# Caxson/mere-fusion

Hardware: AMD Instinct MI355X
Metric: lip-sync frames/sec @256x256 (higher is better)
Workload: dtype bf16x3+f16q; 1 GPU; MuseTalk step 256x256: pe(audio) + UNet(t=0) + VAE decode to uint8 frames, batch=8 latents + Whisper chunks per GPU, inputs resident in HBM (BASELINE.json configs[2]); assumed MuseTalk-v1 / sd-vae-ft-mse architecture, seeded random-init weights; batch_per_gpu=8, parallelism=1 independent replicas, sessions sharded by GPU, no collective

## Files before the change

### mere-fusion_amd/csrc/mf_conv.h

```cpp
#pragma once
#include "mf_common.h"
#include <map>
#include <vector>
#include <utility>

struct ActBuf {
    int C = 0, H = 0, W = 0, halo = 0;
    bf16_t* hi = nullptr;
    bf16_t* lo = nullptr;
    int Hp() const { return H + 2 * halo; }
    int Wp() const { return W + 2 * halo; }
    int64_t per_batch() const { return (int64_t)Hp() * Wp() * C; }
};

struct ActView {
    const ActBuf* buf = nullptr;
    int coff = 0;
    int C = 0;
};

#define MF_MAX_PHASE 9

struct ConvPhase {
    int goff_begin;
// ... 4 lines not shown
    int64_t ws_off;
};

struct ConvArgs {
    const bf16_t* x_hi; const bf16_t* x_lo;
    const bf16_t* w_hi; const bf16_t* w_lo;
    const float* bias;
    const bf16_t* r_hi; const bf16_t* r_lo;
    bf16_t* y_hi; bf16_t* y_lo;
    const int* goff;
    int M, N, Npad;
    int HqWq, Wq;
    uint32_t dv_hw_mul, dv_hw_shr, dv_w_mul, dv_w_shr;
    uint32_t dv_t_mul, dv_t_shr, dv_s_mul, dv_s_shr;
    int64_t xb; int xi, xj;
    int64_t yb; int yi, yj;
    int64_t rb; int ri, rj;
    int act;
    int res_after_act;
    int tiles_m, tiles_n;
    unsigned long long* dbg;
    int m_fastest;
    int ld;
    int wide_store;
    int goff_total;
    int zgroups, zheads;
    int64_t zx_b, zx_h, zw, zy_b, zy_h;
    float* ws;
    int64_t ws_split, wsb; int wsi, wsj;
    double* gn_out; int gn_out_cpg, gn_out_groups;
    double* ln_out; const double* ln_in; const float* ln_cs; float ln_inv_c, ln_eps;
    ConvPhase ph[MF_MAX_PHASE];
};

struct HaloArgs {
    const bf16_t* x_hi; const bf16_t* x_lo;
    const bf16_t* w_hi; const bf16_t* w_lo;
    const float* bias;
    const bf16_t* r_hi; const bf16_t* r_lo;
    bf16_t* y_hi; bf16_t* y_lo;
    int batch, H, W, N, Npad, n_slices;
    int in_halo, in_hp, in_wp, x_ld;
    int64_t xb;
    int64_t yb; int yi, yj;
    int64_t rb; int ri, rj;
    int act;
    int res_from_halo;
    int patches_x, patches_per_img, n_patches, tiles_n;
    float* ws; int64_t ws_split; int nsplit;
    unsigned long long* dbg;
    int q;
    double* gn_out; int gn_out_cpg, gn_out_groups;
    int wide_store;
};
struct HaloTile { int ph, bn, wgm, wgn; };

struct ThinArgs {
    const bf16_t* x_hi; const bf16_t* x_lo;
    const bf16_t* w;
    const float* bias;
    bf16_t* y_hi; bf16_t* y_lo;
    int batch, H, W, N;
    int pad, in_halo, in_hp, in_wp, x_ld;
    int64_t xb, yb; int yi, yj;
    int act;
};
bool mf_thin_supported(int k, int stride, int cin, int cout);
int mf_thin_nks(int k, int cin);
void mf_thin_pack(const float* w, const float* scale, int cout, int cin, int k, bool x3, std::vector<bf16_t>& dst);
int mf_thin_launch(const ThinArgs& a, int k, int stride, int cin, int cout, bool x3, hipStream_t s);
HaloTile mf_halo_pick_tile(int H, int W, int N, int batch, int cin = 0);
int mf_halo_launch(const HaloArgs& a, const HaloTile& t, bool x3, hipStream_t s);
HaloTile mf_halo_w_pick_tile(int H, int W, int N, int batch, int cin = 0);
int mf_halo_w_launch(const HaloArgs& a, const HaloTile& t, bool x3, hipStream_t s, int phase = -1);
struct ConvTile { int bm, bn, wgm, wgn, nsplit; };
struct ConvTuned { ConvTile tile; int ld; };

struct ConvPlan {
    mf_conv2d_desc d{};
    int precision = 0;
    int cin_pad = 0;
    int out_h = 0, out_w = 0;
    int Hq = 0, Wq = 0;
    int nphase = 1;
    int Npad = 0;
    int BK = 64;
    bf16_t* w_hi = nullptr;
    bf16_t* w_lo = nullptr;
    float* bias = nullptr;
    int* goff = nullptr;
    double* out_stats = nullptr; int out_stats_groups = 0;
    const float* ln_gamma = nullptr; const float* ln_beta = nullptr;
    float* ln_cs = nullptr; const double* ln_in = nullptr; float ln_eps = 1e-5f;
    double* ln_out = nullptr;
    bool q_small_maps = false;
    bool q = false;
    bool halo = false;
    bool thin = false;
    bf16_t* up_hi = nullptr;
    bf16_t* up_lo = nullptr;
    ConvPlan* alt = nullptr;
    int n_slices = 0;
    int groups_cap = 1;
    hipEvent_t prof_mid = nullptr;
    float* ws = nullptr;
    int64_t ws_cap = 0;
    std::vector<void*> retired;
    struct Tap {
        int dy, dx;
        std::vector<std::pair<int, int>> src;
    };
    std::vector<std::vector<Tap>> phase_taps;
    std::vector<int> phase_oy, phase_ox;
    int out_step = 1;
    int in_step_h = 1, in_step_w = 1;
    int in_halo_need = 0;
    ConvPhase ph[MF_MAX_PHASE]{};
    int goff_total = 0;
    int bound_in_ld = -1, bound_in_wp = -1;
    std::map<int, ConvTuned> tuned;
};

int mf_conv_plan_create(ConvPlan* p, const mf_conv2d_desc& d, const float* weight, const float* bias,
                        const float* bn_gamma, const float* bn_beta, const float* bn_mean,
                        const float* bn_var, int precision);
void mf_conv_plan_destroy(ConvPlan* p);

int mf_conv_bind(ConvPlan* p, const ActBuf& in);

struct ConvLaunchCfg { int family; ConvTile tile; int ld, bk, nphase, stats; bool pinned; };
int mf_conv_resolve(const ConvPlan* p, int batch, int tokens, int stats_groups, ConvLaunchCfg* c);
bool mf_conv_tuned_valid(const ConvTuned& c, int precision, int act);
int mf_conv_pin(ConvPlan* p, int batch, const ConvTuned& c);
void mf_conv_kernel_name(const ConvPlan* p, int batch, char* buf, int cap);
ConvTile mf_conv_pick_tile(const ConvPlan* p, int batch);
int mf_conv_tune(ConvPlan* p, const ActView& in, const ActView& out, const ActView& res, int batch, hipStream_t stream);
int mf_conv_tune_lookup(ConvPlan* p, const ActView& in, int batch);
bool mf_autotune_enabled();
double mf_conv_flops(const ConvPlan* p, int batch);

struct GroupedGemm {
    const bf16_t* x_hi; const bf16_t* x_lo; int64_t zx_b, zx_h; int x_row;
    bf16_t* y_hi; bf16_t* y_lo; int64_t zy_b, zy_h; int y_row;
    int M, groups, heads;
};
int mf_gemm_grouped_launch(ConvPlan* p, const GroupedGemm& g, hipStream_t stream);

int mf_q_split_count(const ConvPlan* p, int batch);
// ... 6 lines not shown
```

### mere-fusion_amd/csrc/mf_conv.hip

```cpp
#include "mf_conv.h"
#include <dlfcn.h>
#include <cmath>
#include <cstdlib>
#include <cstring>
#include <algorithm>
#include <map>
#include <set>
#include <string>
#include <type_traits>

typedef __attribute__((ext_vector_type(8))) __bf16 bf16x8;
typedef __attribute__((ext_vector_type(4))) float f32x4;
typedef __attribute__((ext_vector_type(4))) unsigned int u32x4;
typedef __attribute__((ext_vector_type(8))) _Float16 f16x8;
typedef __attribute__((ext_vector_type(8))) int i32x8;
typedef __attribute__((ext_vector_type(4))) int i32x4;

template <int BK>
__device__ __forceinline__ int swz(int row) {
    return BK == 32 ? (((row >> 2) & 1) << 1) : (((row >> 1) & 3) << 1);
}
template <int BK>
__device__ __forceinline__ int tile_off(int row, int kg) {
    return row * (BK * 2) + ((kg ^ swz<BK>(row)) << 4);
// ... 1747 lines not shown
        ha.x_hi = ib.hi + in.coff; ha.x_lo = x3 ? ib.lo + in.coff : nullptr;
        ha.w_hi = p->w_hi; ha.w_lo = p->w_lo; ha.bias = p->bias;
        ha.batch = batch; ha.H = p->out_h; ha.W = p->out_w; ha.N = p->d.cout; ha.Npad = p->Npad; ha.n_slices = p->n_slices;
        ha.in_halo = ib.halo; ha.in_hp = ib.Hp(); ha.in_wp = ib.Wp(); ha.x_ld = ib.C; ha.xb = ib.per_batch();
        const int64_t yb0 = ((int64_t)ob.halo * ob.Wp() + ob.halo) * ob.C + out.coff;
        ha.y_hi = ob.hi + yb0; ha.y_lo = x3 ? ob.lo + yb0 : nullptr;
        ha.yb = ob.per_batch(); ha.yi = ob.Wp() * ob.C; ha.yj = ob.C;
        if (res.buf) {
            const ActBuf& rb = *res.buf;
            MF_REQUIRE(rb.H == p->out_h && rb.W == p->out_w && res.C == p->d.cout, "conv: residual view does not match the output");
            if (res.buf == in.buf && res.coff == in.coff && p->d.cin == p->d.cout) {
                ha.res_from_halo = 1;
            } else {
                const int64_t rb0 = ((int64_t)rb.halo * rb.Wp() + rb.halo) * rb.C + res.coff;
                ha.r_hi = rb.hi + rb0; ha.r_lo = x3 ? rb.lo + rb0 : nullptr;
                ha.rb = rb.per_batch(); ha.ri = rb.Wp() * rb.C; ha.rj = rb.C;
            }
        }
        ha.act = p->d.act;
        if (cfg.family == MF_CONV_FAMILY_F16Q) {
            MF_REQUIRE(!ha.res_from_halo, "conv (f16q): residual-from-input is not built for this format");
            if (cfg.stats == MF_CONV_STATS_EPILOGUE) {
                ha.gn_out = p->out_stats; ha.gn_out_cpg = p->d.cout / p->out_stats_groups; ha.gn_out_groups = p->out_stats_groups;
                *stats_done = true;
            }
            ha.wide_store = out.coff % 8 == 0 && ob.C % 8 == 0 && p->d.cout % 32 == 0;
            const HaloTile qtile{16, 128, 4, 2};
            const int ns = cfg.tile.nsplit;
            if (ns > 1) {
                const int64_t per_split = (int64_t)batch * p->out_h * p->out_w * p->d.cout;
                const int64_t need = per_split * ns;
                if (need > p->ws_cap) {
                    if (p->ws) { p->retired.push_back(p->ws); p->ws = nullptr; p->ws_cap = 0; }
                    MF_HIP(hipMalloc(&p->ws, need * sizeof(float)));
                    p->ws_cap = need;
                }
                HaloArgs hs = ha;
                hs.ws = p->ws; hs.ws_split = per_split; hs.nsplit = ns;
                hs.gn_out = nullptr;
                *stats_done = false;
                int rc = mf_halo_w_launch(hs, qtile, true, stream);
                if (rc) return rc;
                ConvArgs e{};
                e.ws = p->ws; e.ws_split = per_split; e.bias = p->bias; e.N = p->d.cout; e.act = p->d.act;
                e.y_hi = ha.y_hi; e.y_lo = ha.y_lo; e.yb = ha.yb; e.yi = ha.yi; e.yj = ha.yj;
                e.r_hi = ha.r_hi; e.r_lo = ha.r_lo; e.rb = ha.rb; e.ri = ha.ri; e.rj = ha.rj;
                const int64_t total = (int64_t)batch * p->out_h * p->out_w * (p->d.cout / 4);
                MF_REQUIRE(total < 0x7fffffffll, "conv: split-K combine over %lld channel quads (32-bit thread index)", (long long)total);
                if (launch_combine_stats(p, e, ns, p->out_h, p->out_w, batch, stream)) *stats_done = true;
                else hipLaunchKernelGGL(k_splitk_epilogue, dim3((unsigned)((total + 255) / 256)), dim3(256), 0, stream, e, ns, p->out_h, p->out_w, (int)total, epi_div(e, p->out_h, p->out_w));
                MF_HIP(hipGetLastError());
                return MF_OK;
            }
            return mf_halo_w_launch(ha, qtile, true, stream);
        }
        if (cfg.family == MF_CONV_FAMILY_HALO_W) return mf_halo_w_launch(ha, HaloTile{cfg.tile.bm, cfg.tile.bn, cfg.tile.wgm, cfg.tile.wgn}, x3, stream);
        {
            const int ns = cfg.tile.nsplit;
            if (cfg.family == MF_CONV_FAMILY_HALO_W_SPLIT) {
                const int64_t per_split = (int64_t)batch * p->out_h * p->out_w * p->d.cout;
                const int64_t need = per_split * ns;
                if (need > p->ws_cap) {
                    if (p->ws) { p->retired.push_back(p->ws); p->ws = nullptr; p->ws_cap = 0; }
                    MF_HIP(hipMalloc(&p->ws, need * sizeof(float)));
                    p->ws_cap = need;
                }
                HaloArgs hs = ha;
                hs.ws = p->ws; hs.ws_split = per_split; hs.nsplit = ns;
                hs.res_from_halo = 0;
                int rc = mf_halo_w_launch(hs, HaloTile{16, 256, 2, 4}, x3, stream);
                if (rc) return rc;
                ConvArgs e{};
                e.ws = p->ws; e.ws_split = per_split; e.bias = p->bias; e.N = p->d.cout; e.act = p->d.act;
                e.y_hi = ha.y_hi; e.y_lo = ha.y_lo; e.yb = ha.yb; e.yi = ha.yi; e.yj = ha.yj;
                if (res.buf) {
                    const ActBuf& rb = *res.buf;
                    const int64_t rb0 = ((int64_t)rb.halo * rb.Wp() + rb.halo) * rb.C + res.coff;
                    e.r_hi = rb.hi + rb0; e.r_lo = x3 ? rb.lo + rb0 : nullptr;
                    e.rb = rb.per_batch(); e.ri = rb.Wp() * rb.C; e.rj = rb.C;
                }
                const int64_t total = (int64_t)batch * p->out_h * p->out_w * (p->d.cout / 4);
                MF_REQUIRE(total < 0x7fffffffll, "conv: split-K combine over %lld channel quads (32-bit thread index)", (long long)total);
                if (launch_combine_stats(p, e, ns, p->out_h, p->out_w, batch, stream)) *stats_done = true;
                else hipLaunchKernelGGL(k_splitk_epilogue, dim3((unsigned)((total + 255) / 256)), dim3(256), 0, stream, e, ns, p->out_h, p->out_w, (int)total, epi_div(e, p->out_h, p->out_w));
                MF_HIP(hipGetLastError());
                return MF_OK;
            }
        }
        if (cfg.family == MF_CONV_FAMILY_TWIN) {
            p->alt->prof_mid = p->prof_mid;
            p->alt->out_stats = p->out_stats; p->alt->out_stats_groups = p->out_stats_groups;
            const int rc = conv_launch_impl(p->alt, in, out, res, batch, stream, 0, stats_done);
            p->alt->prof_mid = nullptr;
            return rc;
        }
        return mf_halo_launch(ha, HaloTile{cfg.tile.bm, cfg.tile.bn, cfg.tile.wgm, cfg.tile.wgn}, x3, stream);
    }

    if (cfg.family == MF_CONV_FAMILY_F16Q) {
        MF_REQUIRE(ib.halo >= 1 && !res.buf, "conv (f16q): upsample path needs an input halo and no residual");
        HaloArgs ha{};
        ha.q = 1;
        ha.x_hi = ib.hi + in.coff; ha.x_lo = ib.lo + in.coff;
        ha.bias = p->bias;
        ha.batch = batch; ha.H = p->d.in_h; ha.W = p->d.in_w; ha.N = p->d.cout; ha.Npad = p->Npad; ha.n_slices = p->n_slices;
        ha.in_halo = ib.halo; ha.in_hp = ib.Hp(); ha.in_wp = ib.Wp(); ha.x_ld = ib.C; ha.xb = ib.per_batch();
// ... 471 lines not shown
```

### mere-fusion_amd/csrc/mf_conv_halo2.hip

```cpp
#include "mf_conv.h"
#include <cstdlib>
#include <cstdio>
#include <vector>
#include <algorithm>
#include <type_traits>

typedef __attribute__((ext_vector_type(8))) __bf16 bf16x8;
typedef __attribute__((ext_vector_type(4))) float f32x4;
typedef __attribute__((ext_vector_type(8))) _Float16 f16x8;
typedef __attribute__((ext_vector_type(8))) int i32x8;
typedef __attribute__((ext_vector_type(4))) int i32x4;

namespace {

constexpr int PW = 16;

template <int CK>
__device__ __forceinline__ int hswz(int hx) {
    return CK == 32 ? (((hx >> 2) & 1) << 1) : (((hx >> 1) & 3) << 1);
}

__device__ __forceinline__ int qswz(int r) { return ((r >> 2) & 1) * 3; }

__device__ __forceinline__ float hbf2f(uint32_t h16) { return __uint_as_float(h16 << 16); }
// ... 499 lines not shown
                __syncthreads();
            }
            wbuf ^= 1;
        }
    }

    if (dbg && threadIdx.x == 0) dbg[2] = __builtin_amdgcn_s_memtime();
    float gs[Q ? FN : 1], gq[Q ? FN : 1];
#pragma unroll
    for (int i = 0; i < (Q ? FN : 1); ++i) { gs[i] = 0.f; gq[i] = 0.f; }
    constexpr int FME = SP ? FM / 2 : FM;
    const int erow0 = row0 + (SP && !cons ? FM / 2 : 0);
    if constexpr (SP) {
        f32x4* xch = reinterpret_cast<f32x4*>(smem);
        __syncthreads();
        if (cons) {
#pragma unroll
            for (int i = 0; i < FN; ++i)
#pragma unroll
                for (int jj = 0; jj < FME; ++jj) xch[((wave * FN + i) * FME + jj) * 64 + lane] = acc[i][FME + jj];
        }
        __syncthreads();
        if (!cons) {
#pragma unroll
            for (int i = 0; i < FN; ++i)
#pragma unroll
                for (int jj = 0; jj < FME; ++jj) acc[i][jj] = xch[(((wave - NW) * FN + i) * FME + jj) * 64 + lane];
        }
    }
    if (a.ws) {
#pragma unroll
        for (int j = 0; j < FME; ++j) {
            const int oy = y0 + erow0 + j, ox = x0 + fr;
            if (oy >= a.H || ox >= a.W) continue;
            float* wo = a.ws + (int64_t)blockIdx.y * a.ws_split + (((int64_t)b * a.H + oy) * a.W + ox) * a.N;
#pragma unroll
            for (int i = 0; i < FN; ++i) {
                const int c = n0 + cn0 + i * 16 + fk * 4;
                if (c >= a.N) continue;
                *reinterpret_cast<float4*>(wo + c) = make_float4(acc[i][j][0], acc[i][j][1], acc[i][j][2], acc[i][j][3]);
            }
        }
        return;
    }
    float4 bq[FN];
#pragma unroll
    for (int i = 0; i < FN; ++i) {
        int c = n0 + cn0 + i * 16 + fk * 4;
        c = c < a.Npad - 3 ? c : a.Npad - 4;
        bq[i] = *reinterpret_cast<const float4*>(a.bias + c);
    }
    const bool has_res = a.r_hi != nullptr;
    const int ox = x0 + fr;
    constexpr int JG = (FME * FN * NP <= 32) ? FME : (32 / (FN * NP) >= 1 ? 32 / (FN * NP) : 1);
#pragma unroll
    for (int j0 = 0; j0 < FME; j0 += JG) {
        uint2 rh[JG][FN], rl[JG][FN];
        if (has_res) {
#pragma unroll
            for (int jj = 0; jj < JG; ++jj) {
                const int j = j0 + jj;
                if (j >= FME) break;
                int oy = y0 + erow0 + j, oxc = ox;
                oy = oy < a.H ? oy : a.H - 1; oxc = oxc < a.W ? oxc : a.W - 1;
                const int64_t ro = (int64_t)b * a.rb + (int64_t)oy * a.ri + (int64_t)oxc * a.rj;
#pragma unroll
                for (int i = 0; i < FN; ++i) {
                    int c = n0 + cn0 + i * 16 + fk * 4;
                    c = c < a.N ? c : 0;
                    rh[jj][i] = *reinterpret_cast<const uint2*>(a.r_hi + ro + c);
                    if (X3) rl[jj][i] = *reinterpret_cast<const uint2*>(a.r_lo + ro + c);
                }
            }
        }
#pragma unroll
        for (int jj = 0; jj < JG; ++jj) {
            const int j = j0 + jj;
            if (j >= FME) break;
            const int oy = y0 + erow0 + j;
            const bool row_ok = oy < a.H && ox < a.W;
            const int64_t yo = (int64_t)b * a.yb + (int64_t)oy * a.yi + (int64_t)ox * a.yj;
            constexpr bool W16 = Q && FN % 2 == 0;
            uint2 pk_hi[W16 ? FN : 1], pk_lo[W16 ? FN : 1];
#pragma unroll
            for (int i = 0; i < FN; ++i) {
                const int c = n0 + cn0 + i * 16 + fk * 4;
                float v[4] = {acc[i][j][0] + bq[i].x, acc[i][j][1] + bq[i].y, acc[i][j][2] + bq[i].z, acc[i][j][3] + bq[i].w};
                if (has_res) {
                    v[0] += hbf2f(rh[jj][i].x & 0xffffu); v[1] += hbf2f(rh[jj][i].x >> 16);
                    v[2] += hbf2f(rh[jj][i].y & 0xffffu); v[3] += hbf2f(rh[jj][i].y >> 16);
                    if (X3) {
                        v[0] += hbf2f(rl[jj][i].x & 0xffffu); v[1] += hbf2f(rl[jj][i].x >> 16);
                        v[2] += hbf2f(rl[jj][i].y & 0xffffu); v[3] += hbf2f(rl[jj][i].y >> 16);
                    }
                }
                if (a.act == 1) {
#pragma unroll
                    for (int e = 0; e < 4; ++e) v[e] = fmaxf(v[e], 0.f);
                } else if (a.act == 2) {
#pragma unroll
                    for (int e = 0; e < 4; ++e) v[e] = 1.f / (1.f + __expf(-v[e]));
                }
                if constexpr (W16) {
                    if (a.wide_store) {
                        if (row_ok && c < a.N) {
                            gs[i] += mf_sum4(v[0], v[1], v[2], v[3]);
                            gq[i] += mf_sum4(v[0] * v[0], v[1] * v[1], v[2] * v[2], v[3] * v[3]);
                        }
                        uint32_t h[4], l[4];
#pragma unroll
                        for (int e = 0; e < 4; ++e) { h[e] = hf2bf(v[e]); l[e] = hf2bf(v[e] - hbf2f(h[e])); }
                        pk_hi[i] = make_uint2(h[0] | (h[1] << 16), h[2] | (h[3] << 16));
                        pk_lo[i] = make_uint2(l[0] | (l[1] << 16), l[2] | (l[3] << 16));
                        continue;
                    }
                }
                if (!row_ok || c >= a.N) continue;
                if constexpr (Q) {
                    gs[i] += mf_sum4(v[0], v[1], v[2], v[3]);
                    gq[i] += mf_sum4(v[0] * v[0], v[1] * v[1], v[2] * v[2], v[3] * v[3]);
                }
                uint32_t h[4];
#pragma unroll
                for (int e = 0; e < 4; ++e) h[e] = hf2bf(v[e]);
                *reinterpret_cast<uint2*>(a.y_hi + yo + c) = make_uint2(h[0] | (h[1] << 16), h[2] | (h[3] << 16));
                if (X3) {
                    uint32_t l[4];
#pragma unroll
                    for (int e = 0; e < 4; ++e) l[e] = hf2bf(v[e] - hbf2f(h[e]));
                    *reinterpret_cast<uint2*>(a.y_lo + yo + c) = make_uint2(l[0] | (l[1] << 16), l[2] | (l[3] << 16));
                }
            }
            if constexpr (W16) {
                if (a.wide_store) {
#pragma unroll
                    for (int i = 0; i + 1 < FN; i += 2) {
                        hstore_pair16(a.y_hi, yo, n0 + cn0 + i * 16, fk, pk_hi[i], pk_hi[i + 1], a.N, row_ok);
                        if (X3) hstore_pair16(a.y_lo, yo, n0 + cn0 + i * 16, fk, pk_lo[i], pk_lo[i + 1], a.N, row_ok);
                    }
                }
            }
        }
    }
    if constexpr (Q) {
        if (a.gn_out) {
            __shared__ float s_gn[NW + NPW][FN * 4][2];
#pragma unroll
            for (int i = 0; i < FN; ++i)
#pragma unroll
                for (int off = 1; off < 16; off <<= 1) { gs[i] += __shfl_xor(gs[i], off); gq[i] += __shfl_xor(gq[i], off); }
            if (fr == 0) {
#pragma unroll
                for (int i = 0; i < FN; ++i) { s_gn[wave][i * 4 + fk][0] = gs[i]; s_gn[wave][i * 4 + fk][1] = gq[i]; }
            }
            __syncthreads();
            const int qpg = a.gn_out_cpg >> 2;
            const int ng = BN / a.gn_out_cpg;
            if (tid < 2 * ng) {
                const int gl = tid >> 1, m = tid & 1;
                double acc_d = 0.0;
                for (int k = 0; k < qpg; ++k) {
                    const int qd = gl * qpg + k;
                    const int wn = qd / (FN * 4), sl = qd - wn * (FN * 4);
#pragma unroll
                    for (int wm = 0; wm < WGM; ++wm) acc_d += (double)s_gn[wn * WGM + wm][sl][m] + (SP ? (double)s_gn[NW + wn * WGM + wm][sl][m] : 0.0);
                }
                const int g = n0 / a.gn_out_cpg + gl;
                if (g < a.gn_out_groups) atomicAdd(a.gn_out + 2 * ((size_t)b * a.gn_out_groups + g) + m, acc_d);
            }
        }
    }
    if (dbg) {
        asm volatile("s_waitcnt vmcnt(0)" ::: "memory");
        if (threadIdx.x == 0) dbg[3] = __builtin_amdgcn_s_memtime();
    }
}

namespace {

template <int PH, int BN, int WGM, int WGN, bool X3, int TR, int PHASE = -1, int HS = 2, bool Q = false, bool SP = false>
int halo_w_launch_cfg(const HaloArgs& a, hipStream_t s) {
    static bool attr_done = false;
    auto kern = k_conv3x3_halo_w<PH, BN, WGM, WGN, X3, TR, PHASE, HS, Q, SP>;
    if (!attr_done) {
        MF_HIP(hipFuncSetAttribute(reinterpret_cast<const void*>(kern),
                                   hipFuncAttributeMaxDynamicSharedMemorySize, (Q ? 158 : 160) * 1024));
        attr_done = true;
    }
    constexpr int CK = X3 ? 32 : 64, RPC = 1024 / (CK * 2), NP = X3 ? 2 : 1;
    constexpr int HCH = ((PH + 2) * (PW + 2) + RPC - 1) / RPC;
    const size_t lds = (size_t)HS * NP * HCH * 1024 + (size_t)(Q ? 4 : 2) * TR * NP * BN * CK * 2;
    static const bool dbg_times = mf_debug_has("times");
    HaloArgs aa = a;
    const size_t nwg = (size_t)a.n_patches * a.tiles_n * (a.nsplit > 1 ? a.nsplit : 1);
    if (dbg_times && nwg <= 65536) {
        static unsigned long long* dbg_buf = nullptr;
        if (!dbg_buf) MF_HIP(hipMalloc(&dbg_buf, (size_t)4 * 65536 * sizeof(unsigned long long)));
        aa.dbg = dbg_buf;
    }
    hipLaunchKernelGGL(kern, dim3(a.n_patches * a.tiles_n, a.nsplit > 1 ? a.nsplit : 1), dim3((WGM * WGN + (SP ? 4 : 0)) * 64), lds, s, aa);
    MF_HIP(hipGetLastError());
    if (aa.dbg) {
        static int reports = 0;
        if (++reports > 3 && reports <= 6) {
            MF_HIP(hipStreamSynchronize(s));
            std::vector<unsigned long long> t(4 * nwg);
            MF_HIP(hipMemcpy(t.data(), aa.dbg, t.size() * sizeof(t[0]), hipMemcpyDeviceToHost));
            unsigned long long lo = ~0ull, hi = 0;
            std::vector<double> d[3], start, end;
            for (size_t w = 0; w < nwg; ++w) {
                lo = std::min(lo, t[4 * w]); hi = std::max(hi, t[4 * w + 3]);
                for (int k = 0; k < 3; ++k) d[k].push_back((double)(t[4 * w + k + 1] - t[4 * w + k]));
            }
            for (size_t w = 0; w < nwg; ++w) { start.push_back((double)(t[4 * w] - lo)); end.push_back((double)(t[4 * w + 3] - lo)); }
            auto med = [](std::vector<double> v) { std::sort(v.begin(), v.end()); return v[v.size() / 2]; };
            auto mx = [](const std::vector<double>& v) { return *std::max_element(v.begin(), v.end()); };
            fprintf(stderr, "[MF_DEBUG=times halo_w<%d,%d,%d,%d>] %zu WGs, %d slices: span %.1f; prologue med %.1f max %.1f; loop med %.1f max %.1f; "
                            "epilogue (to store acks) med %.1f max %.1f; WG start med %.1f max %.1f; WG end med %.1f (s_memtime ticks)\n",
                    PH, BN, WGM, WGN, nwg, a.n_slices, (hi - lo) * 1.0, med(d[0]), mx(d[0]), med(d[1]), mx(d[1]), med(d[2]),
                    mx(d[2]), med(start), mx(start), med(end));
        }
    }
    return MF_OK;
}

template <int PH, int BN, int WGM, int WGN, int TR, int PHASE = -1>
int halo_w_launch_prec(const HaloArgs& a, bool x3, hipStream_t s) {
    return x3 ? halo_w_launch_cfg<PH, BN, WGM, WGN, true, TR, PHASE>(a, s) : halo_w_launch_cfg<PH, BN, WGM, WGN, false, TR, PHASE>(a, s);
}
}

int mf_halo_w_launch(const HaloArgs& a0, const HaloTile& t, bool x3, hipStream_t s, int phase) {
    HaloArgs a = a0;
    a.patches_x = (a.W + PW - 1) / PW;
    const int patches_y = (a.H + t.ph - 1) / t.ph;
    a.patches_per_img = a.patches_x * patches_y;
    a.n_patches = a.batch * a.patches_per_img;
    a.tiles_n = (a.N + t.bn - 1) / t.bn;
    if (a.q) {
        if (t.ph != 16 || t.bn != 128 || t.wgm != 4 || (phase >= 0 && a.nsplit > 1)) { mf_set_error("halo conv (f16 + FP6 format): plain 3x3 layers and unsplit upsample phases on the 16 x 16 x 128 tile only"); return MF_ERR_INVALID; }
        switch (phase) {
            case 0: return halo_w_launch_cfg<16, 128, 2, 2, true, 1, 0, 2, true, true>(a, s);
            case 1: return halo_w_launch_cfg<16, 128, 2, 2, true, 1, 1, 2, true, true>(a, s);
            case 2: return halo_w_launch_cfg<16, 128, 2, 2, true, 1, 2, 2, true, true>(a, s);
            case 3: return halo_w_launch_cfg<16, 128, 2, 2, true, 1, 3, 2, true, true>(a, s);
            default: return halo_w_launch_cfg<16, 128, 2, 2, true, 1, -1, 2, true, true>(a, s);
        }
    }
    if (phase >= 0) { mf_set_error("halo conv (LDS weights): upsample phases exist in the f16 + FP6 format only"); return MF_ERR_INVALID; }
    if (t.ph == 16 && t.bn == 256 && t.wgm == 2) return halo_w_launch_prec<16, 256, 2, 4, 1>(a, x3, s);
    if (t.ph == 16 && t.bn == 128 && t.wgm == 4) return halo_w_launch_prec<16, 128, 4, 2, 1>(a, x3, s);
    if (t.ph == 16 && t.bn == 128 && t.wgm == 2 && t.wgn == 2)
        return x3 ? halo_w_launch_cfg<16, 128, 2, 2, true, 1, -1, 1>(a, s) : halo_w_launch_cfg<16, 128, 2, 2, false, 1, -1, 1>(a, s);
    mf_set_error("halo conv (LDS weights): no kernel for patch %dx16, BN %d", t.ph, t.bn);
    return MF_ERR_INVALID;
}

HaloTile mf_halo_w_pick_tile(int H, int W, int N, int batch, int cin) {
    auto wgs = [&](int ph, int bn) { return batch * ((H + ph - 1) / ph) * ((W + PW - 1) / PW) * ((N + bn - 1) / bn); };
    if (N < 64) return HaloTile{0, 0, 0, 0};
    const bool big_map = H * W >= 64 * 64;
    if (N % 256 == 0 && (big_map || cin >= 512) && wgs(16, 256) >= 256) return HaloTile{16, 256, 2, 4};
    if (N % 128 == 0 && big_map && wgs(16, 128) >= 512) return HaloTile{16, 128, 2, 2};
    if (N % 128 == 0 && big_map && wgs(16, 128) >= 256) return HaloTile{16, 128, 4, 2};
    if (N >= 256 && N % 128 != 0 && N % 64 == 0 && H * W >= 32 * 32 && wgs(16, 128) >= 480) return HaloTile{16, 128, 4, 2};
    return HaloTile{0, 0, 0, 0};
}
```

### mere-fusion_amd/csrc/mf_musetalk.hip

```cpp
#include "mf_nn.h"
#include "mf_aux.h"
#include <algorithm>
#include <cmath>
#include <cstdlib>
#include <cstring>
#include <functional>
#include <map>
#include <set>
#include <memory>
#include <string>
#include <tuple>
#include <vector>

namespace {

typedef std::function<int(int, hipStream_t)> Op;

static int gn_silu_to_q(const ActView& x, const float* dg, const float* db, int groups, float eps, double* st, float* scale, float* shift, const ActBuf& tq, int B,
                        hipStream_t s, bool have_stats, const float* post, bool fuse) {
    const ActBuf& xb = *x.buf;
    if (fuse && (xb.H * xb.W) % 64 == 0) {
        if (!have_stats) { const int rc = mf_groupnorm_stats(x, groups, st, B, s); if (rc) return rc; }
        return mf_affine_silu_to_act_q(x, scale, shift, 1, tq, B, s, post, st, dg, db, groups, eps);
    }
// ... 426 lines not shown
        if (!g0 || !hA || !hB || !nb || !qkv || !ao || !kv || !gg) return MF_ERR_HIP;
        const std::string t = p + ".transformer_blocks.0";
        int rc;
        if ((rc = gn(p + ".norm", x, ActView{g0, 0, C}, groups, 1e-6f, false))) return rc;
        if ((rc = conv(p + ".proj_in", ActView{g0, 0, C}, ActView{hA, 0, C}, C, C, 1, 1, 0, 0, ActView{}))) return rc;
        double *st1 = ln_slot(hA), *st2 = ln_slot(hB), *st3 = ln_slot(hA);
        const bool fold = st1 && st2 && st3;
        if (fold) { last_plan->ln_out = st1; if ((rc = ln_fold_next(t + ".norm1", C, st1))) return rc; }
        else if ((rc = ln(t + ".norm1", ActView{hA, 0, C}, ActView{nb, 0, C}))) return rc;
        {
            const float *wq = T(t + ".attn1.to_q.weight", (int64_t)C * C), *wk = T(t + ".attn1.to_k.weight", (int64_t)C * C),
                        *wv = T(t + ".attn1.to_v.weight", (int64_t)C * C);
            if (!wq || !wk || !wv) return MF_ERR_INVALID;
            std::vector<float> w((size_t)3 * C * C);
            std::copy(wq, wq + (size_t)C * C, w.begin());
            std::copy(wk, wk + (size_t)C * C, w.begin() + (size_t)C * C);
            std::copy(wv, wv + (size_t)C * C, w.begin() + (size_t)2 * C * C);
            if ((rc = linear_raw(w.data(), nullptr, fold ? ActView{hA, 0, C} : ActView{nb, 0, C}, ActView{qkv, 0, 3 * C}, C, 3 * C, ActView{}))) return rc;
        }
        if ((rc = attention(ActView{qkv, 0, C}, ActView{qkv, C, C}, ActView{qkv, 2 * C, C}, ActView{ao, 0, C}, heads))) return rc;
        if ((rc = conv(t + ".attn1.to_out.0", ActView{ao, 0, C}, ActView{hB, 0, C}, C, C, 1, 1, 0, 0, ActView{hA, 0, C}))) return rc;
        if (fold) { last_plan->ln_out = st2; if ((rc = ln_fold_next(t + ".norm2", C, st2))) return rc; }
        else if ((rc = ln(t + ".norm2", ActView{hB, 0, C}, ActView{nb, 0, C}))) return rc;
        if ((rc = conv(t + ".attn2.to_q", fold ? ActView{hB, 0, C} : ActView{nb, 0, C}, ActView{qkv, 0, C}, C, C, 1, 1, 0, 0, ActView{}, 0, nullptr, 1.f, false))) return rc;
        ActView kk{kv, 0, C}, vv{kv, C, C};
        {
            const float *wk = T(t + ".attn2.to_k.weight", (int64_t)C * X), *wv = T(t + ".attn2.to_v.weight", (int64_t)C * X);
            if (!wk || !wv) return MF_ERR_INVALID;
            if (kv_all && kv_off + 2 * C <= kv_all->C && ctx.buf == kv_ctx.buf) {
                kv_w.insert(kv_w.end(), wk, wk + (size_t)C * X);
                kv_w.insert(kv_w.end(), wv, wv + (size_t)C * X);
                kk = ActView{kv_all, kv_off, C}; vv = ActView{kv_all, kv_off + C, C};
                kv_off += 2 * C;
            } else {
                std::vector<float> w((size_t)2 * C * X);
                std::copy(wk, wk + (size_t)C * X, w.begin());
                std::copy(wv, wv + (size_t)C * X, w.begin() + (size_t)C * X);
                if ((rc = linear_raw(w.data(), nullptr, ctx, ActView{kv, 0, 2 * C}, X, 2 * C, ActView{}))) return rc;
            }
        }
        if (kk.buf == kv_all && kv_op >= 0 && !kv_joined) { join_here(kv_op); kv_joined = true; }
        if ((rc = attention(ActView{qkv, 0, C}, kk, vv, ActView{ao, 0, C}, heads))) return rc;
        if ((rc = conv(t + ".attn2.to_out.0", ActView{ao, 0, C}, ActView{hA, 0, C}, C, C, 1, 1, 0, 0, ActView{hB, 0, C}))) return rc;
        if (fold) { last_plan->ln_out = st3; if ((rc = ln_fold_next(t + ".norm3", C, st3))) return rc; }
        else if ((rc = ln(t + ".norm3", ActView{hA, 0, C}, ActView{nb, 0, C}))) return rc;
        if ((rc = conv(t + ".ff.net.0.proj", fold ? ActView{hA, 0, C} : ActView{nb, 0, C}, ActView{gg, 0, 4 * C}, C, 8 * C, 1, 1, 0, 5, ActView{}))) return rc;
        if ((rc = conv(t + ".ff.net.2", ActView{gg, 0, 4 * C}, ActView{hB, 0, C}, 4 * C, C, 1, 1, 0, 0, ActView{hA, 0, C}))) return rc;
        return conv(p + ".proj_out", ActView{hB, 0, C}, y, C, C, 1, 1, 0, 0, x);
    }

#ifndef MF_UP_Q_MIN_WG
#define MF_UP_Q_MIN_WG 256
#endif
    int upsample_conv(const std::string& name, ActView x, ActView out, int C) {
        static const bool on = [] { const char* e = getenv("MF_CONV_Q"); return !e || atoi(e) != 0; }();
        const int H = x.buf->H, W = x.buf->W;
        if (!(on && q_allowed && precision == MF_PREC_BF16X3 && C % 128 == 0 && x.C == C && x.coff % 8 == 0 && H * W >= 32 * 32 &&
              (int64_t)cap * ((H + 15) / 16) * ((W + 15) / 16) * (C / 128) >= MF_UP_Q_MIN_WG))
            return conv(name, x, out, C, C, 3, 1, 1, 0, ActView{}, 1);
        const float* w = T(name + ".weight", (int64_t)C * C * 9);
        const float* b = T(name + ".bias", C);
        if (!w || !b) return MF_ERR_INVALID;
        ActBuf* tq = tmp("up.q", C, H, W, 1);
        if (!tq) return MF_ERR_HIP;
        std::vector<float> ones((size_t)cap * C, 1.f), zeros((size_t)cap * C, 0.f);
        float *d1 = upload(ones.data(), ones.size()), *d0 = upload(zeros.data(), zeros.size());
        if (!d1 || !d0) return MF_ERR_HIP;
        mf_conv2d_desc d{};
        d.cin = C; d.cout = C; d.kh = d.kw = 3; d.stride_h = d.stride_w = 1; d.pad_h = d.pad_w = 1; d.in_h = H; d.in_w = W; d.upsample = 1;
        ConvPlan* p = new_plan();
        int rc = mf_conv_plan_create(p, d, w, b, nullptr, nullptr, nullptr, nullptr, MF_PREC_F16Q);
        if (rc) return rc;
        if ((rc = mf_conv_bind(p, *tq))) return rc;
        stats_forget(out.buf);
        const ActBuf* tqc = tq;
        const ActView tv{tq, 0, C};
        push(name + " (input -> f16 + FP6)", "k_affine_silu_to_q (identity)", 0.0, [=](int B, hipStream_t s) { return mf_affine_silu_to_act_q(x, d1, d0, 0, *tqc, B, s); });
        char kn[96];
        mf_conv_kernel_name(p, cap, kn, sizeof(kn));
        push(name, kn, mf_conv_flops(p, 1), [=](int B, hipStream_t s) { return mf_conv_launch(p, tv, out, ActView{}, B, s); });
        stats_remember(p, out);
        return MF_OK;
    }

    int hoist_kv_begin(ActView ctx, int total) {
        if (total <= 0) return MF_OK;
        kv_all = buf(total, ctx.buf->H, ctx.buf->W, 0);
        if (!kv_all) return MF_ERR_HIP;
        kv_ctx = ctx; kv_off = 0; kv_w.clear();
        push("cross-attention k | v of every block", "(placeholder)", 0.0, [](int, hipStream_t) { return MF_OK; });
        kv_op = (int)ops.size() - 1;
        mark_side(kv_op);
        kv_joined = false;
        return MF_OK;
    }
    int hoist_kv_finish() {
        if (!kv_all) return MF_OK;
        if (kv_off != kv_all->C) { err = "hoisted k | v width does not match the blocks that were built"; return MF_ERR_INVALID; }
        const int X = kv_ctx.C;
        int rc = linear_raw(kv_w.data(), nullptr, kv_ctx, ActView{kv_all, 0, kv_off}, X, kv_off, ActView{});
        if (rc) return rc;
        ops[kv_op] = std::move(ops.back()); ops.pop_back();
        info[kv_op].kernel = info.back().kernel; info[kv_op].flops_per_frame = info.back().flops_per_frame;
        info[kv_op].name = "fused linear " + std::to_string(X) + "->" + std::to_string(kv_off) + " (cross-attention k | v of every block)";
        info.pop_back();
        tunables.back().op = kv_op;
        kv_w.clear(); kv_w.shrink_to_fit();
        return MF_OK;
    }

    int linear_raw(const float* w, const float* b, ActView in, ActView out, int cin, int cout, ActView res) {
        mf_conv2d_desc d{};
        d.cin = cin; d.cout = cout; d.kh = d.kw = 1; d.stride_h = d.stride_w = 1; d.residual = res.buf ? 1 : 0;
        d.in_h = in.buf->H; d.in_w = in.buf->W;
        ConvPlan* p = new_plan();
        ln_apply_fold(p);
        int rc = mf_conv_plan_create(p, d, w, b, nullptr, nullptr, nullptr, nullptr, precision);
        ln_finish_fold(p);
        if (rc) return rc;
        if ((rc = mf_conv_bind(p, *in.buf))) return rc;
        last_plan = p;
        char kn[96];
        mf_conv_kernel_name(p, cap, kn, sizeof(kn));
        push("fused linear " + std::to_string(cin) + "->" + std::to_string(cout), kn, mf_conv_flops(p, 1),
             [p, in, out, res](int B, hipStream_t s) { return mf_conv_launch(p, in, out, res, B, s); });
        tunables.push_back(Tunable{p, in, out, res, (int)ops.size() - 1});
        return MF_OK;
    }

// ... 379 lines not shown
    ActBuf* out_buf = nullptr;
};

extern "C" int mf_vae_create(const mf_vae_config* c, const mf_tensor* weights, int n_weights, int precision, int max_batch,
                             mf_vae** out) {
    MF_REQUIRE(c && weights && out && n_weights > 0 && max_batch > 0, "vae_create: bad argument");
    MF_REQUIRE(c->n_blocks >= 1 && c->n_blocks <= 4 && c->scaling_factor > 0.f, "vae_create: bad config");
    *out = nullptr;
    std::unique_ptr<mf_vae> h(new mf_vae());
    h->cfg = *c;
    Net& net = h->net;
    int rc = net.init(weights, n_weights, precision, max_batch, c->norm_num_groups);
    if (rc) return rc;
    net.q_allowed = true;
    const int nb = c->n_blocks, L = c->layers_per_block, G = c->norm_num_groups, Z = c->latent_channels;
    const int* boc = c->block_out_channels;
    int s = c->sample_size, ch = boc[nb - 1];
    h->in_lat = net.buf(Z, s, s, 1);
    ActBuf *pq = net.buf(Z, s, s, 1), *x0 = net.buf(ch, s, s, 1), *x1 = net.buf(ch, s, s, 1);
    if (!h->in_lat || !pq || !x0 || !x1) { mf_set_error("%s", net.err.c_str()); return MF_ERR_HIP; }
    NET_TRY(net.conv("post_quant_conv", ActView{h->in_lat, 0, h->in_lat->C}, ActView{pq, 0, Z}, Z, Z, 1, 1, 0, 0, ActView{}, 0, nullptr, 1.f / c->scaling_factor));
    NET_TRY(net.conv("decoder.conv_in", ActView{pq, 0, pq->C}, ActView{x0, 0, ch}, Z, ch, 3, 1, 1, 0, ActView{}));
    NET_TRY(net.resnet("decoder.mid_block.resnets.0", ActView{x0, 0, ch}, ActView{x1, 0, ch}, ch, ch, G, 1e-6f, nullptr));
    {
        const std::string a = "decoder.mid_block.attentions.0";
        ActBuf *g0 = net.tmp("va.gn", ch, s, s, 0), *qkv = net.tmp("va.qkv", 3 * ch, s, s, 0), *ao = net.tmp("va.ao", ch, s, s, 0);
        if (!g0 || !qkv || !ao) { mf_set_error("%s", net.err.c_str()); return MF_ERR_HIP; }
        NET_TRY(net.gn(a + ".group_norm", ActView{x1, 0, ch}, ActView{g0, 0, ch}, G, 1e-6f, false));
        const float *wq = net.T(a + ".to_q.weight", (int64_t)ch * ch), *wk = net.T(a + ".to_k.weight", (int64_t)ch * ch), *wv = net.T(a + ".to_v.weight", (int64_t)ch * ch);
        const float *bq = net.T(a + ".to_q.bias", ch), *bk = net.T(a + ".to_k.bias", ch), *bv = net.T(a + ".to_v.bias", ch);
        if (!wq || !wk || !wv || !bq || !bk || !bv) { mf_set_error("%s", net.err.c_str()); return MF_ERR_INVALID; }
        std::vector<float> w((size_t)3 * ch * ch), b((size_t)3 * ch);
        std::copy(wq, wq + (size_t)ch * ch, w.begin()); std::copy(wk, wk + (size_t)ch * ch, w.begin() + (size_t)ch * ch);
        std::copy(wv, wv + (size_t)ch * ch, w.begin() + (size_t)2 * ch * ch);
        std::copy(bq, bq + ch, b.begin()); std::copy(bk, bk + ch, b.begin() + ch); std::copy(bv, bv + ch, b.begin() + 2 * ch);
        NET_TRY(net.linear_raw(w.data(), b.data(), ActView{g0, 0, ch}, ActView{qkv, 0, 3 * ch}, ch, 3 * ch, ActView{}));
        NET_TRY(net.attention(ActView{qkv, 0, ch}, ActView{qkv, ch, ch}, ActView{qkv, 2 * ch, ch}, ActView{ao, 0, ch}, 1));
        NET_TRY(net.conv(a + ".to_out.0", ActView{ao, 0, ch}, ActView{x0, 0, ch}, ch, ch, 1, 1, 0, 0, ActView{x1, 0, ch}));
    }
    NET_TRY(net.resnet("decoder.mid_block.resnets.1", ActView{x0, 0, ch}, ActView{x1, 0, ch}, ch, ch, G, 1e-6f, nullptr));
    ActView x{x1, 0, ch};
    for (int b = 0; b < nb; ++b) {
        const int co = boc[nb - 1 - b];
        for (int i = 0; i < L + 1; ++i) {
            ActBuf* y = net.buf(co, s, s, 1);
            if (!y) { mf_set_error("%s", net.err.c_str()); return MF_ERR_HIP; }
            NET_TRY(net.resnet("decoder.up_blocks." + std::to_string(b) + ".resnets." + std::to_string(i), x, ActView{y, 0, co}, ch, co, G, 1e-6f, nullptr));
            ch = co;
            x = ActView{y, 0, co};
        }
        if (b < nb - 1) {
            ActBuf* y = net.buf(ch, 2 * s, 2 * s, 1);
            if (!y) { mf_set_error("%s", net.err.c_str()); return MF_ERR_HIP; }
            NET_TRY(net.upsample_conv("decoder.up_blocks." + std::to_string(b) + ".upsamplers.0.conv", x, ActView{y, 0, ch}, ch));
            s *= 2;
            x = ActView{y, 0, ch};
        }
    }
    h->out_buf = net.buf(c->out_channels, s, s, 1);
    if (!h->out_buf) { mf_set_error("%s", net.err.c_str()); return MF_ERR_HIP; }
    NET_TRY(net.gn_conv_tail("decoder.conv_norm_out", "decoder.conv_out", x, ActView{h->out_buf, 0, c->out_channels}, ch, c->out_channels, G, 1e-6f));
    *out = h.release();
    return MF_OK;
}

extern "C" int mf_vae_decode_latents(mf_vae* h, const float* latents, uint8_t* frames, float* image_f32, int batch, void* stream) {
    MF_REQUIRE(h && latents && (frames || image_f32), "vae_decode_latents: null argument");
    MF_REQUIRE(batch > 0 && batch <= h->net.cap, "vae_decode_latents: batch %d exceeds the handle's max_batch %d", batch, h->net.cap);
    hipStream_t s = (hipStream_t)stream;
    int rc;
    if ((rc = mf_nchw_to_act(latents, h->cfg.latent_channels, *h->in_lat, batch, s))) return rc;
    if ((rc = h->net.run(batch, s))) return rc;
    const ActView o{h->out_buf, 0, h->cfg.out_channels};
    if (image_f32 && (rc = mf_act_to_nchw(o, image_f32, batch, s))) return rc;
    if (frames && (rc = mf_vae_post_u8(o, frames, batch, s))) return rc;
    return MF_OK;
}

extern "C" int mf_vae_num_ops(const mf_vae* h) { return h ? (int)h->net.ops.size() : 0; }
extern "C" int mf_vae_op_info(const mf_vae* h, int i, char* name, int ncap, char* kernel, int kcap, double* flops_per_frame) {
    MF_REQUIRE(h, "vae_op_info: null handle");
    return h->net.op_info(i, name, ncap, kernel, kcap, flops_per_frame);
}
extern "C" int mf_vae_profile(mf_vae* h, int batch, int iters, float* ms_per_op, void* stream) {
    MF_REQUIRE(h && ms_per_op && batch > 0 && batch <= h->net.cap && iters > 0, "vae_profile: bad argument");
    return h->net.profile(batch, iters, ms_per_op, (hipStream_t)stream);
}
extern "C" int mf_vae_tune(mf_vae* h, int batch, void* stream) {
    MF_REQUIRE(h && batch >= 1 && batch <= h->net.cap, "vae_tune: batch %d exceeds the capacity %d", batch, h ? h->net.cap : 0);
    return h->net.tune(batch, (hipStream_t)stream);
}
extern "C" void mf_vae_destroy(mf_vae* h) { delete h; }


struct mf_vae_encoder {
    mf_vae_config cfg{};
    Net net;
    ActBuf* in_img = nullptr;
    ActBuf* out_buf = nullptr;
    int image_size = 0;
};

extern "C" int mf_vae_encoder_create(const mf_vae_config* c, const mf_tensor* weights, int n_weights, int precision, int max_batch,
                                     mf_vae_encoder** out) {
    MF_REQUIRE(c && weights && out && n_weights > 0 && max_batch > 0, "vae_encoder_create: bad argument");
    MF_REQUIRE(c->n_blocks >= 1 && c->n_blocks <= 4, "vae_encoder_create: bad config");
    *out = nullptr;
// ... 76 lines not shown
```

Baseline: 454.8 frames/s.

## Emit FP6-quantized operand from producer halo conv epilogue for upsample convs

```diff
diff --git a/mere-fusion_amd/csrc/mf_conv.h b/mere-fusion_amd/csrc/mf_conv.h
--- a/mere-fusion_amd/csrc/mf_conv.h
+++ b/mere-fusion_amd/csrc/mf_conv.h
@@ -80,6 +80,9 @@
     int q;
     double* gn_out; int gn_out_cpg, gn_out_groups;
     int wide_store;
+    bf16_t* q_hi; bf16_t* q_lo;
+    int64_t qb; int qi, qj;
+    int q_only;
 };
 struct HaloTile { int ph, bn, wgm, wgn; };
 
@@ -122,6 +125,7 @@
     float* ln_cs = nullptr; const double* ln_in = nullptr; float ln_eps = 1e-5f;
     double* ln_out = nullptr;
     bool q_small_maps = false;
+    const ActBuf* q_out = nullptr; bool q_out_only = false;
     bool q = false;
     bool halo = false;
     bool thin = false;
diff --git a/mere-fusion_amd/csrc/mf_conv.hip b/mere-fusion_amd/csrc/mf_conv.hip
--- a/mere-fusion_amd/csrc/mf_conv.hip
+++ b/mere-fusion_amd/csrc/mf_conv.hip
@@ -1823,6 +1823,15 @@
                 MF_HIP(hipGetLastError());
                 return MF_OK;
             }
+            if (p->q_out) {
+                const ActBuf& qb = *p->q_out;
+                MF_REQUIRE(ha.wide_store && qb.hi && qb.lo && qb.C == p->d.cout && qb.H == p->out_h && qb.W == p->out_w && p->d.cout % 32 == 0,
+                           "conv (f16q): the second output needs an operand buffer of the output's geometry and 16-byte stores");
+                const int64_t q0 = ((int64_t)qb.halo * qb.Wp() + qb.halo) * qb.C;
+                ha.q_hi = qb.hi + q0; ha.q_lo = qb.lo + q0;
+                ha.qb = qb.per_batch(); ha.qi = qb.Wp() * qb.C; ha.qj = qb.C;
+                ha.q_only = p->q_out_only ? 1 : 0;
+            }
             return mf_halo_w_launch(ha, qtile, true, stream);
         }
         if (cfg.family == MF_CONV_FAMILY_HALO_W) return mf_halo_w_launch(ha, HaloTile{cfg.tile.bm, cfg.tile.bn, cfg.tile.wgm, cfg.tile.wgn}, x3, stream);
diff --git a/mere-fusion_amd/csrc/mf_conv_halo2.hip b/mere-fusion_amd/csrc/mf_conv_halo2.hip
--- a/mere-fusion_amd/csrc/mf_conv_halo2.hip
+++ b/mere-fusion_amd/csrc/mf_conv_halo2.hip
@@ -575,6 +575,14 @@
     }
     const bool has_res = a.r_hi != nullptr;
     const int ox = x0 + fr;
+    constexpr bool QOUT = Q && SP && PHASE < 0;
+    constexpr int QSTR = BN + 4;
+    static_assert(!QOUT || PH * PW * QSTR * 4 <= HS * STAGE + 4 * WROW, "the fp32 tile must fit the dynamic LDS block");
+    float* const qstage = reinterpret_cast<float*>(smem);
+    const bool qout = QOUT && a.q_hi != nullptr;
+    if constexpr (QOUT) {
+        if (qout) __syncthreads();
+    }
     constexpr int JG = (FME * FN * NP <= 32) ? FME : (32 / (FN * NP) >= 1 ? 32 / (FN * NP) : 1);
 #pragma unroll
     for (int j0 = 0; j0 < FME; j0 += JG) {
@@ -635,6 +643,10 @@
                         for (int e = 0; e < 4; ++e) { h[e] = hf2bf(v[e]); l[e] = hf2bf(v[e] - hbf2f(h[e])); }
                         pk_hi[i] = make_uint2(h[0] | (h[1] << 16), h[2] | (h[3] << 16));
                         pk_lo[i] = make_uint2(l[0] | (l[1] << 16), l[2] | (l[3] << 16));
+                        if constexpr (QOUT) {
+                            if (qout) *reinterpret_cast<float4*>(qstage + ((erow0 + j) * PW + fr) * QSTR + cn0 + i * 16 + fk * 4) =
+                                make_float4(hbf2f(h[0]) + hbf2f(l[0]), hbf2f(h[1]) + hbf2f(l[1]), hbf2f(h[2]) + hbf2f(l[2]), hbf2f(h[3]) + hbf2f(l[3]));
+                        }
                         continue;
                     }
                 }
@@ -655,12 +667,60 @@
                 }
             }
             if constexpr (W16) {
-                if (a.wide_store) {
+                if (a.wide_store && !(QOUT && a.q_only)) {
 #pragma unroll
                     for (int i = 0; i + 1 < FN; i += 2) {
                         hstore_pair16(a.y_hi, yo, n0 + cn0 + i * 16, fk, pk_hi[i], pk_hi[i + 1], a.N, row_ok);
                         if (X3) hstore_pair16(a.y_lo, yo, n0 + cn0 + i * 16, fk, pk_lo[i], pk_lo[i + 1], a.N, row_ok);
                     }
+                }
+            }
+        }
+    }
+    if constexpr (QOUT) {
+        if (qout) {
+            __syncthreads();
+            typedef float v16f __attribute__((ext_vector_type(16)));
+            typedef _Float16 v32h __attribute__((ext_vector_type(32)));
+            typedef unsigned v6u __attribute__((ext_vector_type(6)));
+            typedef unsigned v16u __attribute__((ext_vector_type(16)));
+#pragma unroll 1
+            for (int it = 0; it < PH * PW * (BN / 32) / ((NW + NPW) * 64); ++it) {
+                const int item = tid + it * (NW + NPW) * 64, blk = item % (BN / 32), pl = item / (BN / 32);
+                const float* sp = qstage + pl * QSTR + blk * 32;
+                v16f le, lod;
+                v16u hbits;
+                float mh = 0.f, ml = 0.f;
+#pragma unroll
+                for (int q4 = 0; q4 < 8; ++q4) {
+                    const float4 f = *reinterpret_cast<const float4*>(sp + 4 * q4);
+                    const float fv[4] = {f.x, f.y, f.z, f.w};
+#pragma unroll
+                    for (int e = 0; e < 4; ++e) {
+                        const int k = 4 * q4 + e;
+                        const float v = fv[e];
+                        const _Float16 h = (_Float16)v;
+                        const float vhk = (float)h, vlk = v - vhk;
+                        mh = fmaxf(mh, fabsf(vhk)); ml = fmaxf(ml, fabsf(vlk));
+                        if (k & 1) lod[k >> 1] = vlk; else le[k >> 1] = vlk;
+                        const uint32_t hb = __builtin_bit_cast(uint16_t, h);
+                        if (k & 1) hbits[k >> 1] |= hb << 16; else hbits[k >> 1] = hb;
+                    }
+                }
+                const uint32_t bl = max((__float_as_uint(ml) >> 23) & 0xffu, 2u) - 2u, bh = max((__float_as_uint(mh) >> 23) & 0xffu, 2u) - 2u;
+                const v6u ql = __builtin_amdgcn_cvt_scalef32_2xpk16_fp6_f32(le, lod, __uint_as_float(bl << 23));
+                const v6u qh = __builtin_amdgcn_cvt_scalef32_pk32_fp6_f16(__builtin_bit_cast(v32h, hbits), __uint_as_float(bh << 23));
+                const int oy = y0 + pl / PW, oxq = x0 + pl % PW, c0 = n0 + blk * 32;
+                if (oy < a.H && oxq < a.W && c0 < a.N) {
+                    const int64_t qo = (int64_t)b * a.qb + (int64_t)oy * a.qi + (int64_t)oxq * a.qj + c0;
+                    uint4* dh = reinterpret_cast<uint4*>(a.q_hi + qo);
+                    uint4* dl = reinterpret_cast<uint4*>(a.q_lo + qo);
+#pragma unroll
+                    for (int q4 = 0; q4 < 4; ++q4) dh[q4] = make_uint4(hbits[4 * q4], hbits[4 * q4 + 1], hbits[4 * q4 + 2], hbits[4 * q4 + 3]);
+                    dl[0] = make_uint4(ql[0], ql[1], ql[2], ql[3]);
+                    dl[1] = make_uint4(ql[4], ql[5], bl, 0u);
+                    dl[2] = make_uint4(qh[0], qh[1], qh[2], qh[3]);
+                    dl[3] = make_uint4(qh[4], qh[5], bh, 0u);
                 }
             }
         }
@@ -762,6 +822,7 @@
     a.tiles_n = (a.N + t.bn - 1) / t.bn;
     if (a.q) {
         if (t.ph != 16 || t.bn != 128 || t.wgm != 4 || (phase >= 0 && a.nsplit > 1)) { mf_set_error("halo conv (f16 + FP6 format): plain 3x3 layers and unsplit upsample phases on the 16 x 16 x 128 tile only"); return MF_ERR_INVALID; }
+        if (phase >= 0 && (a.q_hi || a.q_only)) { mf_set_error("halo conv (f16 + FP6 format): the second output exists on plain 3x3 launches only"); return MF_ERR_INVALID; }
         switch (phase) {
             case 0: return halo_w_launch_cfg<16, 128, 2, 2, true, 1, 0, 2, true, true>(a, s);
             case 1: return halo_w_launch_cfg<16, 128, 2, 2, true, 1, 1, 2, true, true>(a, s);
@@ -770,6 +831,7 @@
             default: return halo_w_launch_cfg<16, 128, 2, 2, true, 1, -1, 2, true, true>(a, s);
         }
     }
+    if (a.q_hi || a.q_only) { mf_set_error("halo conv (LDS weights): the second output exists in the f16 + FP6 format only"); return MF_ERR_INVALID; }
     if (phase >= 0) { mf_set_error("halo conv (LDS weights): upsample phases exist in the f16 + FP6 format only"); return MF_ERR_INVALID; }
     if (t.ph == 16 && t.bn == 256 && t.wgm == 2) return halo_w_launch_prec<16, 256, 2, 4, 1>(a, x3, s);
     if (t.ph == 16 && t.bn == 128 && t.wgm == 4) return halo_w_launch_prec<16, 128, 4, 2, 1>(a, x3, s);
diff --git a/mere-fusion_amd/csrc/mf_musetalk.hip b/mere-fusion_amd/csrc/mf_musetalk.hip
--- a/mere-fusion_amd/csrc/mf_musetalk.hip
+++ b/mere-fusion_amd/csrc/mf_musetalk.hip
@@ -502,7 +502,7 @@
 #ifndef MF_UP_Q_MIN_WG
 #define MF_UP_Q_MIN_WG 256
 #endif
-    int upsample_conv(const std::string& name, ActView x, ActView out, int C) {
+    int upsample_conv(const std::string& name, ActView x, ActView out, int C, bool sole_reader = false) {
         static const bool on = [] { const char* e = getenv("MF_CONV_Q"); return !e || atoi(e) != 0; }();
         const int H = x.buf->H, W = x.buf->W;
         if (!(on && q_allowed && precision == MF_PREC_BF16X3 && C % 128 == 0 && x.C == C && x.coff % 8 == 0 && H * W >= 32 * 32 &&
@@ -522,9 +522,30 @@
         int rc = mf_conv_plan_create(p, d, w, b, nullptr, nullptr, nullptr, nullptr, MF_PREC_F16Q);
         if (rc) return rc;
         if ((rc = mf_conv_bind(p, *tq))) return rc;
+        const bool from_conv = [] { const char* e = getenv("MF_UP_Q_FROM_CONV"); return !e || atoi(e) != 0; }();
+        ConvPlan* prod = nullptr;
+        if (from_conv && x.coff == 0 && x.buf->C == C)
+            for (const StatsSrc& e : stats_srcs)
+                if (e.v.buf == x.buf && e.v.coff == 0 && e.v.C == C && e.p->q && e.p->halo && !e.p->d.upsample && e.p->d.cout == C && !e.p->q_out &&
+                    mf_q_split_count(e.p, cap) == 1)
+                    prod = e.p;
         stats_forget(out.buf);
         const ActBuf* tqc = tq;
         const ActView tv{tq, 0, C};
+        if (prod) {
+            prod->q_out = tq; prod->q_out_only = sole_reader;
+            char kn[96];
+            mf_conv_kernel_name(p, cap, kn, sizeof(kn));
+            push(name, kn, mf_conv_flops(p, 1), [=](int B, hipStream_t s) {
+                if (mf_q_split_count(prod, B) > 1) {
+                    const int rc = mf_affine_silu_to_act_q(x, d1, d0, 0, *tqc, B, s);
+                    if (rc) return rc;
+                }
+                return mf_conv_launch(p, tv, out, ActView{}, B, s);
+            });
+            stats_remember(p, out);
+            return MF_OK;
+        }
         push(name + " (input -> f16 + FP6)", "k_affine_silu_to_q (identity)", 0.0, [=](int B, hipStream_t s) { return mf_affine_silu_to_act_q(x, d1, d0, 0, *tqc, B, s); });
         char kn[96];
         mf_conv_kernel_name(p, cap, kn, sizeof(kn));
@@ -1010,7 +1031,7 @@
         if (b < nb - 1) {
             ActBuf* y = net.buf(ch, 2 * s, 2 * s, 1);
             if (!y) { mf_set_error("%s", net.err.c_str()); return MF_ERR_HIP; }
-            NET_TRY(net.upsample_conv("decoder.up_blocks." + std::to_string(b) + ".upsamplers.0.conv", x, ActView{y, 0, ch}, ch));
+            NET_TRY(net.upsample_conv("decoder.up_blocks." + std::to_string(b) + ".upsamplers.0.conv", x, ActView{y, 0, ch}, ch, true));
             s *= 2;
             x = ActView{y, 0, ch};
         }
```

Result: slower. 446.7 frames/s (-1.8%).
